# lbcb-sci/herro

Hardware: AMD Instinct MI355X
Metric: 4096-bp windows corrected/sec at batch=128 (higher is better)
Workload: dtype f16; 1 GPU; synthetic windows, 4096 bp, 32 overlaps each, batch=128, 1xMI355X per rank (BASELINE configs[2]); batch=128, window=4096, overlaps=32, batches_per_launch_group=32, streams_per_gpu=2, distinct_windows_cycled=16384, precision=5, total_windows=165760, strong_leg_windows=0

## Files before the change

herro_amd/csrc/pileup.hip:

```cpp
#include <hip/hip_runtime.h>
#include <stdint.h>

#include <cstdio>
#include <cstdlib>
#include <mutex>
#include <set>
#include <type_traits>

#include "job_dev.h"
#include "pileup_core.h"

namespace herro {

namespace {

constexpr uint32_t NONE = 0xffffffffu;
constexpr uint32_t RF_LEFT = 0x80000000u;
constexpr uint32_t ROWCAP = HERRO_TILE;
constexpr uint32_t SCAP = 128;
constexpr uint32_t QEVCAP = 2048;

template <int NT>
__device__ __forceinline__ uint32_t blk_scan(uint32_t v, uint32_t* total, uint32_t* s_wave ) {
  const int lane = threadIdx.x & 63, wave = threadIdx.x >> 6;
// ... 930 lines not shown
#pragma unroll
    for (int q = 0; q < 5; q++) cw[q] = cg == 0 ? cnt8[q][0] : (cg == 1 ? cnt8[q][1] : (cg == 2 ? cnt8[q][2] : cnt8[q][3]));
    const uint4 adj = *reinterpret_cast<const uint4*>(s_adj + seg * 16u + cg * 4u);
    const uint32_t adjw[4] = {adj.x, adj.y, adj.z, adj.w};
    uint32_t supb = 0, consw = 0;
#pragma unroll
    for (int q4 = 0; q4 < 4; q4++) {
      uint32_t c5[5];
#pragma unroll
      for (int q = 0; q < 4; q++) c5[q] = ((cw[q] >> (8 * q4)) & 0xffu) + ((adjw[q4] >> (5 * q)) & 31u);
      c5[4] = ((cw[4] >> (8 * q4)) & 0xffu) - (adjw[q4] >> 20);
      const uint32_t thresh = (uint32_t)((double)HERRO_ROWS * 0.1);
      uint32_t ns = 0;
#pragma unroll
      for (int q = 0; q < 5; q++) ns += c5[q] >= thresh ? 1u : 0u;
      if (ns >= 2 && seg * 16u + cg * 4u + q4 < nrows) supb |= 1u << q4;
      uint32_t c0 = c5[0], i0 = 0;
#pragma unroll
      for (uint32_t q = 1; q < 5; q++) if (c5[q] > c0) { c0 = c5[q]; i0 = q; }
      uint32_t c1 = 0, i1 = 5;
      bool have = false;
#pragma unroll
      for (uint32_t q = 0; q < 5; q++)
        if (q != i0 && (!have || c5[q] > c1)) { c1 = c5[q]; i1 = q; have = true; }
      const uint32_t tb0 = (tgw >> (q4 * 8)) & 0xffu;
      const uint32_t cons_v = (c0 < 2u || (c0 == c1 && (i0 == tb0 || i1 == tb0))) ? tb0 : i0;
      consw |= cons_v << (q4 * 8);
    }
    if (aux) *reinterpret_cast<uint32_t*>(J.cons_tmp + wd.row_off + r0 + seg * 16u + cg * 4u) = consw;
    if (supb) atomicOr(&s_supbits[(seg * 16u + cg * 4u) >> 5], supb << ((seg * 16u + cg * 4u) & 31u));
  }
  __syncthreads();
  PROF_MARK(J, 3, 5);
  if (aux && tid < 64) {
    const uint32_t bits = tid < ROWCAP / 32 ? s_supbits[tid] : 0u;
    const uint32_t inc = wscan_incl((uint32_t)__popc(bits));
    uint32_t k = inc - (uint32_t)__popc(bits);
    for (uint32_t m = bits; m; m &= m - 1u) {
      const uint32_t ric = (tid << 5) + (uint32_t)__ffs((int)m) - 1u;
      const uint32_t p = pa + (s_rowinfo[ric] & 0x7fffu), row = r0 + ric;
      J.sup_row[wd.row_off + r0 + k] = row;
      J.sup_pi[wd.row_off + r0 + k] = p | ((row - rop(p)) << 16);
      k++;
    }
    if (tid == 63) J.tile_nsup[tile] = inc;
  }
  PROF_MARK(J, 3, 6);
}

__global__ __launch_bounds__(64) void k_supgather(JobDev J) {
  const uint32_t w = blockIdx.x, lane = threadIdx.x;
  const WinDesc wd = J.win[w];
  const uint32_t Lf = J.win_Lf[w], tile0 = (uint32_t)wd.col_off;
  const uint32_t nch = (Lf + ROWCAP - 1) / ROWCAP;
  uint32_t dst = 0;
  for (uint32_t c0 = 0; c0 < nch; c0 += 64) {
    const uint32_t i = c0 + lane;
    const uint32_t cn = i < nch ? J.tile_nsup[tile0 + i] : 0u;
    const uint32_t inc = wscan_incl(cn);
    const uint32_t my_dst = dst + inc - cn;
    for (uint32_t j = 0; j < 64 && c0 + j < nch; j++) {
      const uint32_t cnt_j = (uint32_t)__builtin_amdgcn_readlane((int)cn, (int)j), dst_j = (uint32_t)__builtin_amdgcn_readlane((int)my_dst, (int)j);
      const uint32_t src = (c0 + j) * ROWCAP;
      if (src == dst_j) continue;
      for (uint32_t k = lane; k < cnt_j; k += 64) {
        const uint32_t a = J.sup_row[wd.row_off + src + k], b = J.sup_pi[wd.row_off + src + k];
        J.sup_row[wd.row_off + dst_j + k] = a;
        J.sup_pi[wd.row_off + dst_j + k] = b;
      }
    }
    dst += wlast(inc);
  }
  if (lane == 0) J.win_nsup[w] = dst;
}

#ifndef HERRO_RW_ICAP
#define HERRO_RW_ICAP 2048
#endif
constexpr uint32_t RW_ICAP = HERRO_RW_ICAP;
#define RI(p) ((p) + ((p) >> 5))
__host__ __device__ inline size_t rows_lds(uint32_t W) { return (size_t)(W + 2 + ((W + 2) >> 5) + 1) * 4; }

constexpr uint32_t RW_SUPCAP = 256;
template <int SP>
__device__ __forceinline__ void rf_slot(const JobDev& J, const CTab* __restrict__ s_ct, const WinDesc& wd, uint32_t Lf, uint32_t half, uint32_t c,
                                        uint32_t srow, uint32_t pj, uint32_t nr, bool have_nr, uint4* __restrict__ out);

template <int NW>
__global__ __launch_bounds__(2 * NW) void k_rows(JobDev J) {
  constexpr int NT = 2 * NW;
  extern __shared__ __attribute__((aligned(16))) uint32_t rw_smem[];
  uint32_t* s_rop = rw_smem;
  uint32_t* s_mrg = rw_smem + rows_lds(J.window_size) / 4;
  __shared__ __attribute__((aligned(16))) CTab s_ct[32];
  __shared__ uint32_t s_adj[RW_ICAP];
  __shared__ __attribute__((aligned(16))) uint8_t s_iv[RW_ICAP];
  __shared__ uint32_t s_rfbase;
  __shared__ uint32_t s_sup[3][RW_SUPCAP];
  __shared__ uint32_t s_wave[NT / 64];
  const uint32_t w = blockIdx.x, tid = threadIdx.x, nw = J.nw;
  const uint32_t half = tid >= (uint32_t)NW ? 1u : 0u, lt = tid - half * NW;
  PROF_BEGIN(J);
  const WinDesc wd = J.win[w];
  const uint32_t Lf = J.win_Lf[w], win_len = wd.win_len;
  const uint32_t tile0 = (uint32_t)wd.col_off;
  {
    constexpr int RL = 17;
    uint32_t rv[RL];
    const uint32_t* __restrict__ rop = J.row_of_pos2 + wd.pos_off;
#pragma unroll
    for (int u = 0; u < RL; u++) rv[u] = rop[min(tid + (uint32_t)u * NT, win_len)];
    if (tid < 32) s_ct[tid] = J.ctab[(uint64_t)w * 32 + tid];
#pragma unroll
    for (int u = 0; u < RL; u++) {
      const uint32_t p = tid + (uint32_t)u * NT;
      if (p <= win_len) s_rop[RI(p)] = rv[u];
    }
  }
  __syncthreads();
  PROF_MARK(J, 6, 0);
  const bool active = lt < nw;
  const uint32_t widx = min(lt, nw - 1u);
  const int32_t P = (int32_t)(widx << 5);
  const uint32_t vm = active ? mask_range(0, (int32_t)win_len - P) : 0u;
  const uint64_t pmax = J.read_n_words + 1;
  const uint32_t tlo = glb_bits(J.read_p0, s_ct[0].q_woff, pmax, (int32_t)wd.tstart + P) & vm;
  const uint32_t thi = glb_bits(J.read_p1, s_ct[0].q_woff, pmax, (int32_t)wd.tstart + P) & vm;
  uint32_t c0[5], c1[5];
  uint32_t nin[5];
  const uint32_t tsym[4] = {vm & ~tlo & ~thi, tlo & ~thi, thi & ~tlo, tlo & thi};
#pragma unroll
  for (int q = 0; q < 4; q++) { c0[q] = half ? 0u : tsym[q]; c1[q] = 0; }
  c0[4] = 0; c1[4] = 0;
  nin[0] = half ? 0u : vm; nin[1] = 0; nin[2] = 0; nin[3] = 0; nin[4] = 0;
  auto sat_add = [&](int q, uint32_t x) { sat2_add(c0[q], c1[q], x); };
  {
    constexpr int UB = 15;
    const uint32_t cb = 1u + UB * half;
    uint32_t M[UB], L[UB], H[UB];
#pragma unroll
    for (int u = 0; u < UB; u++) {
      const uint32_t o = s_ct[cb + u].ow;
      const PlaneRec g = J.cw[(o != NONE ? (uint64_t)o : 0ull) * nw + widx];
      M[u] = g.m; L[u] = g.lo; H[u] = g.hi;
    }
    PROF_MARK(J, 6, 10);
#pragma unroll
    for (int u = 0; u < UB; u++) {
      const CTab& h = s_ct[cb + u];
      const uint32_t tt = h.ow != NONE ? h.t_total : 0u;
      const uint32_t inr = mask_range(h.off - P, h.off + (int32_t)tt - P) & vm;
      const uint32_t Mi = M[u] & inr, Li = L[u] & Mi, Hi = H[u] & Mi;
      sat_add(0, Mi & ~Li & ~Hi);
      sat_add(1, Li & ~Hi);
      sat_add(2, Hi & ~Li);
      sat_add(3, Li & Hi);
      sat_add(4, inr & ~Mi);
      uint32_t x = inr;
#pragma unroll
      for (int b = 0; b < 5; b++) { const uint32_t cy = nin[b] & x; nin[b] ^= x; x = cy; }
    }
  }
  if (half) {
#pragma unroll
    for (int q = 0; q < 5; q++) { s_mrg[(q) * NW + lt] = c0[q]; s_mrg[(5 + q) * NW + lt] = c1[q]; s_mrg[(10 + q) * NW + lt] = nin[q]; }
  }
  __syncthreads();
  if (!half) {
#pragma unroll
    for (int q = 0; q < 5; q++) sat2_merge(c0[q], c1[q], s_mrg[q * NW + lt], s_mrg[(5 + q) * NW + lt]);
    uint32_t cy = 0;
#pragma unroll
    for (int b = 0; b < 5; b++) {
      const uint32_t x = nin[b], y = s_mrg[(10 + b) * NW + lt];
      nin[b] = x ^ y ^ cy;
      cy = (x & y) | (cy & (x ^ y));
    }
  }
  const bool lane0 = !half && active;
  constexpr uint32_t IP_ROWS = (RW_ICAP * 2 + NW * 4 - 1) / (NW * 4);
  static_assert(IP_ROWS + 7 <= 15, "s_mrg holds the insertion rows' positions, five cover planes and two words per lane");
  uint16_t* s_ip = reinterpret_cast<uint16_t*>(s_mrg);
// ... 73 lines not shown
            if (s_ct[c].sdir < 0) code ^= 3u;
          }
          atomicAdd(&s_adj[ir], (1u << (5u * code)) + (inr ? 1u << 20 : 0u));
          s_ip[ir] = (uint16_t)p;
        }
      }
    }
    __syncthreads();
    PROF_MARK(J, 6, 8);
    for (uint32_t i = tid; i < min(RW_ICAP, n_irows - ch0); i += NT) {
      const uint32_t adj = s_adj[i];
      uint32_t cover = 0, p = 0;
      if (adj) {
        p = s_ip[i];
        const uint32_t pw = p >> 5, pb = p & 31u;
        cover = ((s_nin[pw] >> pb) & 1u) | (((s_nin[NW + pw] >> pb) & 1u) << 1) | (((s_nin[2 * NW + pw] >> pb) & 1u) << 2) |
                (((s_nin[3 * NW + pw] >> pb) & 1u) << 3) | (((s_nin[4 * NW + pw] >> pb) & 1u) << 4);
      }
      const uint32_t c5[5] = {adj & 31u, (adj >> 5) & 31u, (adj >> 10) & 31u, (adj >> 15) & 31u, cover - (adj >> 20)};
      uint32_t ns = 0;
#pragma unroll
      for (int q = 0; q < 5; q++) ns += c5[q] >= 3u ? 1u : 0u;
      s_iv[i] = (uint8_t)(vote5(c5, 4u) | ((ns >= 2u ? 1u : 0u) << 7));
      if (ns >= 2u) { atomicOr(&s_insup[p >> 5], 1u << (p & 31u)); atomicAdd(&s_nisup[p >> 5], 1u); }
    }
    __syncthreads();
    PROF_MARK(J, 6, 9);
    if (lane0) { insup = s_insup[lt]; n_isup = s_nisup[lt]; }
    {
      const uint32_t nb = min(RW_ICAP, n_irows - ch0);
      uint32_t* __restrict__ dst = reinterpret_cast<uint32_t*>(J.cons_tmp + wd.row_off + ch0);
      for (uint32_t i = tid; i * 4u < nb; i += NT) dst[i] = reinterpret_cast<const uint32_t*>(s_iv)[i];
    }
  }
  PROF_MARK(J, 6, 3);
  const bool iv_lds = n_irows <= RW_ICAP;
  if (!iv_lds) __syncthreads();
  uint32_t total;
  uint32_t kk = blk_scan<NT>((uint32_t)__popc(supb) + n_isup, &total, s_wave);
  for (uint32_t m = supb | insup; m; m &= m - 1u) {
    const uint32_t k = (uint32_t)__ffs((int)m) - 1u, p = (uint32_t)P + k;
    const uint32_t rp = s_rop[RI(p)];
    uint32_t nr = 0;
#pragma unroll
    for (int i = 0; i < 4; i++) {
      const int32_t q = (int32_t)p - 2 + i;
      if (q >= 0 && q < (int32_t)win_len) nr |= (s_rop[RI((uint32_t)q + 1u)] - s_rop[RI((uint32_t)q)]) << (6 * i);
    }
    if ((supb >> k) & 1u) {
      J.sup_row[wd.row_off + kk] = rp;
      J.sup_pi[wd.row_off + kk] = p;
      J.sup_nr[wd.row_off + kk] = nr;
      if (kk < RW_SUPCAP) { s_sup[0][kk] = rp; s_sup[1][kk] = p; s_sup[2][kk] = nr; }
      kk++;
    }
    if ((insup >> k) & 1u) {
      const uint32_t n_ins = s_rop[RI(p + 1)] - rp - 1u;
      for (uint32_t j = 0; j < n_ins; j++) {
        const uint32_t ir = rp - p + j;
        uint32_t fl;
        if (iv_lds) fl = (uint32_t)s_iv[ir]; else fl = (uint32_t)J.cons_tmp[wd.row_off + ir];
        if (fl & 0x80u) {
          J.sup_row[wd.row_off + kk] = rp + 1u + j;
          J.sup_pi[wd.row_off + kk] = p | ((j + 1u) << 16);
          J.sup_nr[wd.row_off + kk] = nr;
          if (kk < RW_SUPCAP) { s_sup[0][kk] = rp + 1u + j; s_sup[1][kk] = p | ((j + 1u) << 16); s_sup[2][kk] = nr; }
          kk++;
        }
      }
    }
  }
  if (tid == 0) J.win_nsup[w] = total;
  PROF_MARK(J, 6, 4);
  if (J.rf) {
    if (tid == 0) {
      const uint32_t base = atomicAdd(J.rf_alloc, total);
      const bool room = (uint64_t)base + total <= J.rf_cap, ok = room && total <= RW_SUPCAP;
      s_rfbase = ok ? base : NONE;
      J.win_rfbase[w] = ok ? base : (room ? (base | RF_LEFT) : NONE);
    }
    __syncthreads();
    const uint32_t base = s_rfbase;
    if (base != NONE) {
      const uint32_t nslots = total * HERRO_ROWS;
      for (uint32_t sl = tid; sl < nslots; sl += NT) {
        const uint32_t k = sl / HERRO_ROWS, c = sl - k * HERRO_ROWS;
        uint4* __restrict__ out = reinterpret_cast<uint4*>(J.rf + ((uint64_t)base * HERRO_ROWS + sl) * 16);
        if (J.rf_half <= 2u) rf_slot<5>(J, s_ct, wd, Lf, J.rf_half, c, s_sup[0][k], s_sup[1][k], s_sup[2][k], true, out);
        else rf_slot<8>(J, s_ct, wd, Lf, J.rf_half, c, s_sup[0][k], s_sup[1][k], s_sup[2][k], true, out);
      }
    }
    PROF_MARK(J, 6, 5);
  }
}

constexpr int PQ_NT = 256;
constexpr uint32_t RFCAP = 1024;
__host__ __device__ inline size_t quals_lds(uint32_t nw) {
  return (size_t)(HERRO_ROWS - 1) * nw * 4 + (((size_t)(HERRO_ROWS - 1) * nw * 2 + 15) & ~(size_t)15) + (size_t)QEVCAP * 8;
}

template <bool FULL>
__global__ __launch_bounds__(PQ_NT) void k_quals(JobDev J, uint32_t half) {
  extern __shared__ __attribute__((aligned(16))) unsigned char pq_smem[];
  const uint32_t nw = J.nw;
  uint32_t* s_M = reinterpret_cast<uint32_t*>(pq_smem);
  uint16_t* s_rk = reinterpret_cast<uint16_t*>(s_M + (size_t)(HERRO_ROWS - 1) * nw);
  uint2* s_ev = reinterpret_cast<uint2*>(pq_smem + (size_t)(HERRO_ROWS - 1) * nw * 4 + (((size_t)(HERRO_ROWS - 1) * nw * 2 + 15) & ~(size_t)15));
  __shared__ __attribute__((aligned(16))) CTab s_ct[32];
  __shared__ uint32_t s_evl[33];
  __shared__ uint32_t s_rm[RFCAP];
  __shared__ uint32_t s_rr[RFCAP];
  const uint32_t w = blockIdx.x, tid = threadIdx.x, lane = tid & 63u, wave = tid >> 6;
  const uint32_t nsup = J.win_nsup[w], Lf = J.win_Lf[w];
  const WinDesc wd = J.win[w];
  if (tid < 32) s_ct[tid] = J.ctab[(uint64_t)w * 32 + tid];
  if (!FULL && !nsup) return;
  __syncthreads();
  if (tid < 64) {
    const uint32_t ne = (tid >= 1 && tid < 32) ? s_ct[tid].n_ev : 0u;
    const uint32_t inc = wscan_incl(ne);
    if (tid < 32) s_evl[tid] = inc - ne;
    if (tid == 31) s_evl[32] = inc;
  }
  __syncthreads();
  const uint32_t n_events = s_evl[32];
  const bool ev_in_lds = n_events <= QEVCAP;
  const uint32_t span = 2 * half + 1;
  const uint32_t kper = max(1u, RFCAP / span);
  {
    const uint32_t items = (HERRO_ROWS - 1) * nw;
    constexpr int MI = 16;
    uint32_t srow = 0;
    if (!FULL && tid < min(kper, nsup)) srow = J.sup_row[wd.row_off + tid];
    constexpr int EI = QEVCAP / PQ_NT;
    uint2 ev[EI];
    if (ev_in_lds) {
#pragma unroll
      for (int u = 0; u < EI; u++) {
        const uint32_t e = min(tid + u * PQ_NT, n_events ? n_events - 1u : 0u);
        uint32_t lo = 0, hi = 32;
        while (hi - lo > 1) {
          const uint32_t mid = (lo + hi) >> 1;
          if (s_evl[mid] <= e) lo = mid; else hi = mid;
        }
        ev[u] = n_events ? *reinterpret_cast<const uint2*>(J.iev + (uint64_t)s_ct[lo].ev_off + (e - s_evl[lo])) : make_uint2(0, 0);
      }
    }
    for (uint32_t it0 = tid; it0 < items; it0 += MI * PQ_NT) {
      uint32_t mv[MI];
#pragma unroll
      for (int u = 0; u < MI; u++) {
        const uint32_t it = min(it0 + u * PQ_NT, items - 1u);
        const uint32_t c = it / nw, wi = it - c * nw;
        const uint32_t o = s_ct[c + 1].ow;
        mv[u] = J.cw[(o != NONE ? (uint64_t)o : 0ull) * nw + wi].m;
      }
#pragma unroll
      for (int u = 0; u < MI; u++) {
        const uint32_t it = it0 + u * PQ_NT;
        if (it < items) s_M[it] = s_ct[it / nw + 1].ow != NONE ? mv[u] : 0u;
      }
    }
    if (ev_in_lds) {
#pragma unroll
      for (int u = 0; u < EI; u++) if (tid + u * PQ_NT < n_events) s_ev[tid + u * PQ_NT] = ev[u];
    }
    if (!FULL && tid < min(kper, nsup)) s_rr[tid] = srow;
  }
  __syncthreads();
  uint32_t pre_rm = NONE, pre_r = 0;
  const bool pre = !FULL && kper <= PQ_NT && min(kper, nsup) * span <= PQ_NT * 1u;
  if (pre) {
// ... 57 lines not shown
      bool found = false;
      qi = 0;
      while (i > 0) {
        const uint32_t ex = ev_x(i - 1);
        if ((ex & 0xffffu) != p) break;
        if ((ex >> 16) >= j) { qi = ev_y(i - 1) + j - 1u; found = true; break; }
        i--;
      }
      if (!found) return NONE64;
    }
    const int64_t si = (int64_t)q.sbase + (int64_t)q.sdir * (int64_t)qi;
    return min(q.qual_off + (uint64_t)max(si, (int64_t)0), qmax);
  };
  auto run = [&](auto evlds) {
    if (FULL) {
      const uint64_t total = (uint64_t)Lf * HERRO_ROWS;
      for (uint64_t idx0 = tid; idx0 < total; idx0 += 4 * PQ_NT) {
        uint32_t rm[4];
        uint64_t dst[4], src[4];
        uint32_t cc[4];
#pragma unroll
        for (int u = 0; u < 4; u++) {
          const uint64_t idx = min(idx0 + (uint64_t)u * PQ_NT, total - 1);
          cc[u] = (uint32_t)(idx / Lf);
          const uint32_t r = (uint32_t)(idx - (uint64_t)cc[u] * Lf);
          rm[u] = J.rowmap2[wd.row_off + r];
          dst[u] = wd.fin_off + (uint64_t)cc[u] * wd.lub + r;
        }
#pragma unroll
        for (int u = 0; u < 4; u++) src[u] = cell_addr(evlds, cc[u], rm[u] & 0xffffu, rm[u] >> 16);
        uint32_t qv[4];
#pragma unroll
        for (int u = 0; u < 4; u++) qv[u] = J.read_qual[src[u] == NONE64 ? 0 : src[u]];
#pragma unroll
        for (int u = 0; u < 4; u++)
          if (idx0 + (uint64_t)u * PQ_NT < total) J.fin_q[dst[u]] = (uint8_t)(src[u] == NONE64 ? 33u : qv[u]);
      }
    } else {
      for (uint32_t k0 = 0; k0 < nsup; k0 += kper) {
        const uint32_t nk = min(kper, nsup - k0), nrows = nk * span;
        if (k0 == 0 && pre) {
          if (tid < nrows) { s_rr[tid] = pre_r; s_rm[tid] = pre_rm; }
        } else {
          __syncthreads();
          for (uint32_t i = tid; i < nrows; i += PQ_NT) {
            const int64_t r = (int64_t)J.sup_row[wd.row_off + k0 + i / span] + (int64_t)(i % span) - (int64_t)half;
            const bool in = r >= 0 && r < (int64_t)Lf;
            s_rr[i] = (uint32_t)r;
            s_rm[i] = in ? J.rowmap2[wd.row_off + (uint32_t)r] : NONE;
          }
        }
        __syncthreads();
        const uint32_t total = nrows * HERRO_ROWS;
        uint8_t* __restrict__ outp = J.fin_q;
        constexpr int CB = 10;
        for (uint32_t idx0 = tid; idx0 < total; idx0 += CB * PQ_NT) {
          uint64_t dst[CB], src[CB];
          bool live[CB];
#pragma unroll
          for (int u = 0; u < CB; u++) {
            const uint32_t idx = min(idx0 + u * PQ_NT, total - 1u);
            const uint32_t slot = idx / HERRO_ROWS, c = idx - slot * HERRO_ROWS;
            dst[u] = wd.fin_off + (uint64_t)c * wd.lub + s_rr[slot];
            const uint32_t rm = s_rm[slot];
            live[u] = idx0 + u * PQ_NT < total && rm != NONE;
            src[u] = live[u] ? cell_addr(evlds, c, rm & 0xffffu, rm >> 16) : NONE64;
          }
          uint32_t qv[CB];
#pragma unroll
          for (int u = 0; u < CB; u++) qv[u] = J.read_qual[src[u] == NONE64 ? 0 : src[u]];
#pragma unroll
          for (int u = 0; u < CB; u++)
            if (live[u]) outp[dst[u]] = (uint8_t)(src[u] == NONE64 ? 33u : qv[u]);
        }
      }
    }
  };
  if (ev_in_lds) run(std::true_type{}); else run(std::false_type{});
}

constexpr int RQ_NT = 512;

template <int SP>
__device__ __forceinline__ void rf_slot(const JobDev& J, const CTab* __restrict__ s_ct, const WinDesc& wd, uint32_t Lf, uint32_t half, uint32_t c,
                                        uint32_t srow, uint32_t pj, uint32_t nr, bool have_nr, uint4* __restrict__ out) {
  const uint32_t nw = J.nw;
  const uint32_t span = 2 * half + 1, win_len = wd.win_len;
  const uint64_t tq_off = s_ct[0].qual_off + wd.tstart;
  const uint64_t qmax = J.read_qual_bytes ? J.read_qual_bytes - 1 : 0;
  const uint64_t pmax = J.read_n_words + 1;
  constexpr uint64_t NONE64 = ~0ull;
  const uint32_t* __restrict__ rop = J.row_of_pos2 + wd.pos_off;
  const int32_t pc = (int32_t)(pj & 0xffffu);
  const int64_t row0 = (int64_t)srow - (int64_t)half;
  uint32_t rv[SP];
  if (have_nr && half == 2) {
    const uint32_t rc = srow - (pj >> 16);
    rv[2] = rc;
    rv[1] = rc - ((nr >> 6) & 63u);
    rv[0] = rv[1] - (nr & 63u);
    rv[3] = rc + ((nr >> 12) & 63u);
    rv[4] = rv[3] + ((nr >> 18) & 63u);
    if constexpr (SP > 5) { rv[5] = 0; rv[6] = 0; rv[7] = 0; }
  } else {
#pragma unroll
    for (int i = 0; i < SP; i++) rv[i] = rop[(uint32_t)min(max(pc - (int32_t)half + i, 0), (int32_t)win_len)];
  }
  uint32_t rm[SP];
#pragma unroll
  for (int d = 0; d < SP; d++) {
    const int64_t r = row0 + d;
    rm[d] = NONE;
    if ((uint32_t)d < span && r >= 0 && r < (int64_t)Lf) {
      int32_t pp = 0;
      uint32_t rb = 0;
#pragma unroll
      for (int i = 0; i < SP; i++) {
        const int32_t q = pc - (int32_t)half + i;
        if ((uint32_t)i <= 2 * half && q >= 0 && q < (int32_t)win_len && (int64_t)rv[i] <= r) { pp = q; rb = rv[i]; }
      }
      rm[d] = (uint32_t)pp | (((uint32_t)r - rb) << 16);
    }
  }
  uint64_t addr[SP];
  uint32_t tok[SP];
#pragma unroll
  for (int d = 0; d < SP; d++) { addr[d] = NONE64; tok[d] = TOK_NONE; }
  const CTab& q = s_ct[c];
  if (c == 0) {
    const uint64_t tw = s_ct[0].q_woff;
#pragma unroll
    for (int d = 0; d < SP; d++) {
      if (rm[d] == NONE) continue;
      tok[d] = TOK_GAP_F;
      if ((rm[d] >> 16) == 0) {
        const uint32_t tp = wd.tstart + (rm[d] & 0xffffu);
        const uint64_t wi = min(tw + (tp >> 5), pmax);
        addr[d] = min(tq_off + (rm[d] & 0xffffu), qmax);
        tok[d] = ((J.read_p0[wi] >> (tp & 31u)) & 1u) | (((J.read_p1[wi] >> (tp & 31u)) & 1u) << 1);
      }
    }
  } else if (q.ow != NONE) {
    const uint32_t tbase = q.tokc & 0xffu, tgap = q.tokc >> 8;
    uint32_t p0 = NONE;
#pragma unroll
    for (int d = SP - 1; d >= 0; d--) if (rm[d] != NONE) p0 = rm[d] & 0xffffu;
    if (p0 != NONE) {
      const uint32_t w0 = min(p0 >> 5, nw - 1u), w1 = min(w0 + 1u, nw - 1u);
      const PlaneRec* __restrict__ cw = J.cw + (uint64_t)q.ow * nw;
      const uint32_t* __restrict__ cwd = J.cwd + (uint64_t)q.ow * nw;
      const PlaneRec c0 = cw[w0], c1 = cw[w1];
      uint2 dd;
      __builtin_memcpy(&dd, cwd + w0, 8);
      const uint2 d0 = make_uint2(c0.m, dd.x), d1 = make_uint2(c1.m, w1 != w0 ? dd.y : dd.x);
      const uint32_t l0 = c0.lo, l1 = c1.lo, h0 = c0.hi, h1 = c1.hi;
      const uint32_t m0 = d0.x, m1 = d1.x;
      const uint32_t n_ev = q.n_ev;
      const uint4* __restrict__ iev = J.iev + q.ev_off;
      uint32_t qw = d0.y & 0xfffffu, e = d0.y >> 20;
      if (d0.y == 0xffffffffu) {
        qw = 0; e = 0;
        for (uint32_t i = 0; i < w0; i++) qw += (uint32_t)__popc(cw[i].m);
        while (e < n_ev && (iev[e].x & 0xffffu) < (w0 << 5)) { qw += iev[e].x >> 16; e++; }
      }
      uint32_t pl = p0;
      bool ins_row = false;
#pragma unroll
      for (int d = 0; d < SP; d++) if (rm[d] != NONE) { pl = rm[d] & 0xffffu; ins_row = ins_row || (rm[d] >> 16) != 0; }
      const bool quiet = d0.y != 0xffffffffu && d1.y != 0xffffffffu && w1 != w0 && (d1.y >> 20) == e && (pl >> 5) == w0 && !ins_row;
      const uint32_t e_first = e;
      const uint4 none4 = make_uint4(0xffffffffu, 0, 0, 0);
      const uint32_t e_last = n_ev ? n_ev - 1u : 0u;
      uint4 ep0 = iev[min(e, e_last)], ep1 = iev[min(e + 1u, e_last)], ep2 = iev[min(e + 2u, e_last)], ep3 = iev[min(e + 3u, e_last)];
      if (quiet || e >= n_ev) ep0.x = 0xffffffffu;
      if (quiet || e + 1u >= n_ev) ep1.x = 0xffffffffu;
      if (quiet || e + 2u >= n_ev) ep2.x = 0xffffffffu;
      if (quiet || e + 3u >= n_ev) ep3.x = 0xffffffffu;
      auto ev_at = [&](uint32_t i) -> uint4 {
        if (i >= n_ev) return none4;
        const uint32_t o = i - e_first;
        if (o >= 4u) return iev[i];
        const uint4 a = (o & 1u) ? ep1 : ep0, b = (o & 1u) ? ep3 : ep2;
        return (o & 2u) ? b : a;
      };
      uint4 ecur = ep0;
      uint32_t cum = 0;
#pragma unroll
      for (int d = 0; d < SP; d++) {
        if (rm[d] == NONE) continue;
        const uint32_t p = rm[d] & 0xffffu, j = rm[d] >> 16;
        while ((ecur.x & 0xffffu) < p) {
          cum += ecur.x >> 16;
          e++;
          ecur = ev_at(e);
        }
        const bool second = (p >> 5) != w0;
        const uint32_t mw = second ? m1 : m0;
        const uint32_t below = (uint32_t)__popc(mw & ((1u << (p & 31u)) - 1u)) + (second ? (uint32_t)__popc(m0) : 0u);
        const uint32_t mbit = (mw >> (p & 31u)) & 1u;
        const bool inr = p - (uint32_t)q.off < q.t_total;
        uint32_t qi = NONE;
        tok[d] = inr ? tgap : (uint32_t)TOK_NONE;
        if (j == 0) {
          if (inr && mbit) {
            qi = qw + below + cum;
            tok[d] = tbase + ((((second ? l1 : l0) >> (p & 31u)) & 1u) | ((((second ? h1 : h0) >> (p & 31u)) & 1u) << 1));
          }
        } else if ((ecur.x & 0xffffu) == p) {
          uint4 x = ecur;
          uint32_t code = 0;
          for (uint32_t i = e;;) {
            if ((x.x >> 16) >= j) {
              qi = x.y + j - 1u;
              code = j <= 16u ? (((x.z >> (j - 1u)) & 1u) | (((x.z >> (15u + j)) & 1u) << 1)) : 4u;
            }
            if (++i >= n_ev) break;
            x = ev_at(i);
            if ((x.x & 0xffffu) != p) break;
          }
          if (qi != NONE) {
            if (code == 4u) {
              const int32_t si = q.sbase + q.sdir * (int32_t)qi;
              const uint64_t wi = min(q.q_woff + ((uint32_t)si >> 5), pmax);
              code = ((J.read_p0[wi] >> ((uint32_t)si & 31u)) & 1u) | (((J.read_p1[wi] >> ((uint32_t)si & 31u)) & 1u) << 1);
              if (q.sdir < 0) code ^= 3u;
            }
            tok[d] = tbase + code;
          }
        }
        if (qi != NONE) {
          const int64_t si = (int64_t)q.sbase + (int64_t)q.sdir * (int64_t)qi;
          addr[d] = min(q.qual_off + (uint64_t)max(si, (int64_t)0), qmax);
        }
      }
    }
  }
  uint32_t qv[SP];
#pragma unroll
  for (int d = 0; d < SP; d++) qv[d] = J.read_qual[addr[d] == NONE64 ? 0 : addr[d]];
  uint32_t lo = 0, hi = 0, tl = 0, th = 0;
#pragma unroll
  for (int d = 0; d < 4; d++) {
    lo |= (addr[d] == NONE64 ? 33u : qv[d]) << (8 * d);
    tl |= tok[d] << (8 * d);
    if (d + 4 < SP) {
      hi |= (addr[(d + 4) % SP] == NONE64 ? 33u : qv[(d + 4) % SP]) << (8 * d);
      th |= tok[(d + 4) % SP] << (8 * d);
    } else {
      hi |= 33u << (8 * d);
      th |= (uint32_t)TOK_NONE << (8 * d);
    }
  }
  *out = make_uint4(tl, th, lo, hi);
}

template <int SP>
__global__ __launch_bounds__(RQ_NT) void k_rfq(JobDev J, uint32_t half, const uint64_t* __restrict__ sup_off, uint8_t* __restrict__ rf, uint64_t cap, uint32_t have_nr) {
  __shared__ __attribute__((aligned(16))) CTab s_ct[32];
  const uint32_t w = gridDim.x - 1u - blockIdx.x, tid = threadIdx.x;
  PROF_BEGIN(J);
  const uint32_t nsup = J.win_nsup[w], Lf = J.win_Lf[w];
  const bool left_only = (have_nr & 2u) != 0u;
  have_nr &= 1u;
  uint64_t slot0;
  if (left_only) {
    const uint32_t rb = J.win_rfbase[w];
    if (!nsup || rb == NONE || !(rb & RF_LEFT)) return;
    slot0 = rb & ~RF_LEFT;
  } else {
    if (!nsup || sup_off[w] + nsup > cap) return;
    slot0 = sup_off[w];
  }
  const WinDesc wd = J.win[w];
  if (tid < 32) s_ct[tid] = J.ctab[(uint64_t)w * 32 + tid];
  __syncthreads();
  PROF_MARK(J, 5, 0);
  const uint32_t nslots = nsup * HERRO_ROWS;
  const uint64_t out0 = slot0 * HERRO_ROWS;
  for (uint32_t sl = tid; sl < nslots; sl += RQ_NT) {
    const uint32_t k = sl / HERRO_ROWS, c = sl - k * HERRO_ROWS;
    const uint32_t pj = J.sup_pi[wd.row_off + k], srow = J.sup_row[wd.row_off + k];
    const uint32_t nr = have_nr ? J.sup_nr[wd.row_off + k] : 0u;
    rf_slot<SP>(J, s_ct, wd, Lf, half, c, srow, pj, nr, have_nr != 0u, reinterpret_cast<uint4*>(rf + (out0 + sl) * 16));
    PROF_MARK(J, 5, 1);
  }
}

constexpr int PC_NT = 256;
__global__ __launch_bounds__(PC_NT) void k_consensus(JobDev J, const uint64_t* sup_off, const float* base_logits) {
  __shared__ uint32_t s_wave[PC_NT / 64];
  const uint32_t w = blockIdx.x;
  const WinDesc wd = J.win[w];
  const uint32_t Lf = J.win_Lf[w], n_kept = J.win_nkept[w];
  const uint32_t n_alns = n_kept < 30u ? n_kept : 30u;
  uint8_t* seq = J.cons_seq + wd.row_off;
  if (n_alns < 2) {
    if (threadIdx.x == 0) J.cons_len[w] = 0;
    return;
  }
  const float* lg = base_logits + sup_off[w] * 5;
  uint8_t* tmp = J.cons_tmp + wd.row_off;
  const uint32_t nsup = J.win_nsup[w];
  for (uint32_t k = threadIdx.x; k < nsup; k += PC_NT) {
    const float* l5 = lg + (uint64_t)k * 5;
    uint32_t arg = 0;
    float mx = l5[0];
#pragma unroll
    for (uint32_t c = 1; c < 5; c++) {
      const float v = l5[c];
      const bool ge = (v != v) ? true : ((mx != mx) ? false : v >= mx);
      if (ge) { arg = c; mx = v; }
    }
    tmp[J.sup_row[wd.row_off + k]] = (uint8_t)arg;
  }
  __syncthreads();
  const uint32_t ch = (Lf + PC_NT - 1) / PC_NT;
  const uint32_t a = min(threadIdx.x * ch, Lf), b = min(a + ch, Lf);
  uint32_t nout = 0;
  for (uint32_t r = a; r < b; r++) nout += tmp[r] != 4u ? 1u : 0u;
  uint32_t total;
  uint32_t o = blk_scan<PC_NT>(nout, &total, s_wave);
  uint32_t acc = 0, nacc = 0;
  for (uint32_t r = a; r < b; r++) {
    const uint32_t base = tmp[r];
    if (base == 4u) continue;
    const uint32_t ch = ((0x54474341u >> (8u * base)) & 0xffu);
    if ((o & 3u) != 0 && nacc == 0) { seq[o++] = (uint8_t)ch; continue; }
    acc |= ch << (8 * nacc);
    if (++nacc == 4) { *reinterpret_cast<uint32_t*>(seq + o) = acc; o += 4; acc = 0; nacc = 0; }
  }
  for (uint32_t k = 0; k < nacc; k++) seq[o + k] = (uint8_t)(acc >> (8 * k));
  if (threadIdx.x == 0) J.cons_len[w] = total;
}

constexpr uint32_t CP_ICAP = 4096;
constexpr uint32_t CP_OCAP = 6144;
template <int NT, int SPW>
__global__ __launch_bounds__(NT) void k_consensus_p(JobDev J, const uint64_t* sup_off, const float* base_logits) {
  extern __shared__ __attribute__((aligned(16))) uint32_t cp_smem[];
  uint32_t* s_rop = cp_smem;
  __shared__ uint32_t s_v[3][HERRO_MAX_WINDOW / 32];
  __shared__ uint32_t s_im[HERRO_MAX_WINDOW / 32];
  __shared__ __attribute__((aligned(16))) uint8_t s_iv[CP_ICAP];
  __shared__ __attribute__((aligned(16))) uint8_t s_out[CP_OCAP];
  __shared__ uint32_t s_wave[NT / 64];
  const uint32_t w = blockIdx.x, tid = threadIdx.x, nw = J.nw;
  PROF_BEGIN(J);
  const WinDesc wd = J.win[w];
  const uint32_t Lf = J.win_Lf[w], n_kept = J.win_nkept[w], win_len = wd.win_len;
  const uint32_t n_alns = n_kept < 30u ? n_kept : 30u;
  uint8_t* __restrict__ seq = J.cons_seq + wd.row_off;
  if (n_alns < 2) {
    if (tid == 0) J.cons_len[w] = 0;
    return;
  }
  const uint32_t n_irows = Lf - win_len;
  const bool iv_lds = n_irows <= CP_ICAP;
  uint8_t* __restrict__ giv = J.cons_tmp + wd.row_off;
  {
    constexpr int RL = SPW == 4 ? 9 : 17;
    uint32_t rv[RL];
    const uint32_t* __restrict__ rop = J.row_of_pos2 + wd.pos_off;
#pragma unroll
    for (int u = 0; u < RL; u++) rv[u] = rop[min(tid + (uint32_t)u * NT, win_len)];
    uint32_t vv[4] = {0, 0, 0, 0};
    if (tid < nw) {
      const uint32_t* __restrict__ vp = J.vpl + (uint64_t)w * 4 * nw + tid;
      vv[0] = vp[0]; vv[1] = vp[nw]; vv[2] = vp[2 * nw]; vv[3] = vp[3 * nw];
// ... 222 lines not shown
```

Measured before the change: 3.543 million windows/s.

## Share per-row feature plans across columns via LDS in row-feature gather

Row-feature generation now runs in two phases. Each supporting row's position/row mapping (the plan) is computed once per chunk of 64 rows and stored in shared memory, and every column thread reuses it instead of recomputing it. The target column and the other columns get separate specialised paths. The per-column event walk becomes a branch-free accumulation over prefetched events, and quality loads use 32-bit offsets. This removes redundant row-mapping work and divergent loops, at the cost of extra syncthreads per chunk and LDS space reused from the merge buffer.

```diff
diff --git a/herro_amd/csrc/pileup.hip b/herro_amd/csrc/pileup.hip
--- a/herro_amd/csrc/pileup.hip
+++ b/herro_amd/csrc/pileup.hip
@@ -1036,9 +1036,11 @@
 __host__ __device__ inline size_t rows_lds(uint32_t W) { return (size_t)(W + 2 + ((W + 2) >> 5) + 1) * 4; }
 
 constexpr uint32_t RW_SUPCAP = 256;
-template <int SP>
-__device__ __forceinline__ void rf_slot(const JobDev& J, const CTab* __restrict__ s_ct, const WinDesc& wd, uint32_t Lf, uint32_t half, uint32_t c,
-                                        uint32_t srow, uint32_t pj, uint32_t nr, bool have_nr, uint4* __restrict__ out);
+constexpr uint32_t RF_CHUNK = 64;
+constexpr uint32_t rf_pw(int SP) { return (uint32_t)((SP + 2 + 3) & ~3); }
+template <int SP, int NT, class RowSrc>
+__device__ __forceinline__ void rf_window(const JobDev& J, const CTab* __restrict__ s_ct, uint32_t* __restrict__ s_plan, const WinDesc& wd, uint32_t Lf, uint32_t half,
+                                          bool have_nr, uint32_t nsup, uint8_t* __restrict__ rf, uint64_t slot0, RowSrc rows);
 
 template <int NW>
 __global__ __launch_bounds__(2 * NW) void k_rows(JobDev J) {
@@ -1052,6 +1054,8 @@
   __shared__ uint32_t s_rfbase;
   __shared__ uint32_t s_sup[3][RW_SUPCAP];
   __shared__ uint32_t s_wave[NT / 64];
+  static_assert(15 * NW >= (int)(RF_CHUNK * rf_pw(8)) + 3, "s_mrg holds a chunk of row plans");
+  uint32_t* s_plan = rw_smem + ((rows_lds(J.window_size) / 4 + 3) & ~(size_t)3);
   const uint32_t w = blockIdx.x, tid = threadIdx.x, nw = J.nw;
   const uint32_t half = tid >= (uint32_t)NW ? 1u : 0u, lt = tid - half * NW;
   PROF_BEGIN(J);
@@ -1291,13 +1295,9 @@
     __syncthreads();
     const uint32_t base = s_rfbase;
     if (base != NONE) {
-      const uint32_t nslots = total * HERRO_ROWS;
-      for (uint32_t sl = tid; sl < nslots; sl += NT) {
-        const uint32_t k = sl / HERRO_ROWS, c = sl - k * HERRO_ROWS;
-        uint4* __restrict__ out = reinterpret_cast<uint4*>(J.rf + ((uint64_t)base * HERRO_ROWS + sl) * 16);
-        if (J.rf_half <= 2u) rf_slot<5>(J, s_ct, wd, Lf, J.rf_half, c, s_sup[0][k], s_sup[1][k], s_sup[2][k], true, out);
-        else rf_slot<8>(J, s_ct, wd, Lf, J.rf_half, c, s_sup[0][k], s_sup[1][k], s_sup[2][k], true, out);
-      }
+      auto rows = [&](uint32_t k, uint32_t& srow, uint32_t& pj, uint32_t& nr) { srow = s_sup[0][k]; pj = s_sup[1][k]; nr = s_sup[2][k]; };
+      if (J.rf_half <= 2u) rf_window<5, NT>(J, s_ct, s_plan, wd, Lf, J.rf_half, true, total, J.rf, base, rows);
+      else rf_window<8, NT>(J, s_ct, s_plan, wd, Lf, J.rf_half, true, total, J.rf, base, rows);
     }
     PROF_MARK(J, 6, 5);
   }
@@ -1521,14 +1521,10 @@
 constexpr int RQ_NT = 512;
 
 template <int SP>
-__device__ __forceinline__ void rf_slot(const JobDev& J, const CTab* __restrict__ s_ct, const WinDesc& wd, uint32_t Lf, uint32_t half, uint32_t c,
-                                        uint32_t srow, uint32_t pj, uint32_t nr, bool have_nr, uint4* __restrict__ out) {
+__device__ __forceinline__ void rf_plan(const JobDev& J, const WinDesc& wd, uint32_t Lf, uint32_t half, uint32_t srow, uint32_t pj, uint32_t nr, bool have_nr,
+                                        uint32_t* __restrict__ plan) {
   const uint32_t nw = J.nw;
   const uint32_t span = 2 * half + 1, win_len = wd.win_len;
-  const uint64_t tq_off = s_ct[0].qual_off + wd.tstart;
-  const uint64_t qmax = J.read_qual_bytes ? J.read_qual_bytes - 1 : 0;
-  const uint64_t pmax = J.read_n_words + 1;
-  constexpr uint64_t NONE64 = ~0ull;
   const uint32_t* __restrict__ rop = J.row_of_pos2 + wd.pos_off;
   const int32_t pc = (int32_t)(pj & 0xffffu);
   const int64_t row0 = (int64_t)srow - (int64_t)half;
@@ -1561,129 +1557,40 @@
       rm[d] = (uint32_t)pp | (((uint32_t)r - rb) << 16);
     }
   }
-  uint64_t addr[SP];
-  uint32_t tok[SP];
-#pragma unroll
-  for (int d = 0; d < SP; d++) { addr[d] = NONE64; tok[d] = TOK_NONE; }
-  const CTab& q = s_ct[c];
-  if (c == 0) {
-    const uint64_t tw = s_ct[0].q_woff;
-#pragma unroll
-    for (int d = 0; d < SP; d++) {
-      if (rm[d] == NONE) continue;
-      tok[d] = TOK_GAP_F;
-      if ((rm[d] >> 16) == 0) {
-        const uint32_t tp = wd.tstart + (rm[d] & 0xffffu);
-        const uint64_t wi = min(tw + (tp >> 5), pmax);
-        addr[d] = min(tq_off + (rm[d] & 0xffffu), qmax);
-        tok[d] = ((J.read_p0[wi] >> (tp & 31u)) & 1u) | (((J.read_p1[wi] >> (tp & 31u)) & 1u) << 1);
-      }
-    }
-  } else if (q.ow != NONE) {
-    const uint32_t tbase = q.tokc & 0xffu, tgap = q.tokc >> 8;
-    uint32_t p0 = NONE;
-#pragma unroll
-    for (int d = SP - 1; d >= 0; d--) if (rm[d] != NONE) p0 = rm[d] & 0xffffu;
-    if (p0 != NONE) {
-      const uint32_t w0 = min(p0 >> 5, nw - 1u), w1 = min(w0 + 1u, nw - 1u);
-      const PlaneRec* __restrict__ cw = J.cw + (uint64_t)q.ow * nw;
-      const uint32_t* __restrict__ cwd = J.cwd + (uint64_t)q.ow * nw;
-      const PlaneRec c0 = cw[w0], c1 = cw[w1];
-      uint2 dd;
-      __builtin_memcpy(&dd, cwd + w0, 8);
-      const uint2 d0 = make_uint2(c0.m, dd.x), d1 = make_uint2(c1.m, w1 != w0 ? dd.y : dd.x);
-      const uint32_t l0 = c0.lo, l1 = c1.lo, h0 = c0.hi, h1 = c1.hi;
-      const uint32_t m0 = d0.x, m1 = d1.x;
-      const uint32_t n_ev = q.n_ev;
-      const uint4* __restrict__ iev = J.iev + q.ev_off;
-      uint32_t qw = d0.y & 0xfffffu, e = d0.y >> 20;
-      if (d0.y == 0xffffffffu) {
-        qw = 0; e = 0;
-        for (uint32_t i = 0; i < w0; i++) qw += (uint32_t)__popc(cw[i].m);
-        while (e < n_ev && (iev[e].x & 0xffffu) < (w0 << 5)) { qw += iev[e].x >> 16; e++; }
-      }
-      uint32_t pl = p0;
-      bool ins_row = false;
-#pragma unroll
-      for (int d = 0; d < SP; d++) if (rm[d] != NONE) { pl = rm[d] & 0xffffu; ins_row = ins_row || (rm[d] >> 16) != 0; }
-      const bool quiet = d0.y != 0xffffffffu && d1.y != 0xffffffffu && w1 != w0 && (d1.y >> 20) == e && (pl >> 5) == w0 && !ins_row;
-      const uint32_t e_first = e;
-      const uint4 none4 = make_uint4(0xffffffffu, 0, 0, 0);
-      const uint32_t e_last = n_ev ? n_ev - 1u : 0u;
-      uint4 ep0 = iev[min(e, e_last)], ep1 = iev[min(e + 1u, e_last)], ep2 = iev[min(e + 2u, e_last)], ep3 = iev[min(e + 3u, e_last)];
-      if (quiet || e >= n_ev) ep0.x = 0xffffffffu;
-      if (quiet || e + 1u >= n_ev) ep1.x = 0xffffffffu;
-      if (quiet || e + 2u >= n_ev) ep2.x = 0xffffffffu;
-      if (quiet || e + 3u >= n_ev) ep3.x = 0xffffffffu;
-      auto ev_at = [&](uint32_t i) -> uint4 {
-        if (i >= n_ev) return none4;
-        const uint32_t o = i - e_first;
-        if (o >= 4u) return iev[i];
-        const uint4 a = (o & 1u) ? ep1 : ep0, b = (o & 1u) ? ep3 : ep2;
-        return (o & 2u) ? b : a;
-      };
-      uint4 ecur = ep0;
-      uint32_t cum = 0;
-#pragma unroll
-      for (int d = 0; d < SP; d++) {
-        if (rm[d] == NONE) continue;
-        const uint32_t p = rm[d] & 0xffffu, j = rm[d] >> 16;
-        while ((ecur.x & 0xffffu) < p) {
-          cum += ecur.x >> 16;
-          e++;
-          ecur = ev_at(e);
-        }
-        const bool second = (p >> 5) != w0;
-        const uint32_t mw = second ? m1 : m0;
-        const uint32_t below = (uint32_t)__popc(mw & ((1u << (p & 31u)) - 1u)) + (second ? (uint32_t)__popc(m0) : 0u);
-        const uint32_t mbit = (mw >> (p & 31u)) & 1u;
-        const bool inr = p - (uint32_t)q.off < q.t_total;
-        uint32_t qi = NONE;
-        tok[d] = inr ? tgap : (uint32_t)TOK_NONE;
-        if (j == 0) {
-          if (inr && mbit) {
-            qi = qw + below + cum;
-            tok[d] = tbase + ((((second ? l1 : l0) >> (p & 31u)) & 1u) | ((((second ? h1 : h0) >> (p & 31u)) & 1u) << 1));
-          }
-        } else if ((ecur.x & 0xffffu) == p) {
-          uint4 x = ecur;
-          uint32_t code = 0;
-          for (uint32_t i = e;;) {
-            if ((x.x >> 16) >= j) {
-              qi = x.y + j - 1u;
-              code = j <= 16u ? (((x.z >> (j - 1u)) & 1u) | (((x.z >> (15u + j)) & 1u) << 1)) : 4u;
-            }
-            if (++i >= n_ev) break;
-            x = ev_at(i);
-            if ((x.x & 0xffffu) != p) break;
-          }
-          if (qi != NONE) {
-            if (code == 4u) {
-              const int32_t si = q.sbase + q.sdir * (int32_t)qi;
-              const uint64_t wi = min(q.q_woff + ((uint32_t)si >> 5), pmax);
-              code = ((J.read_p0[wi] >> ((uint32_t)si & 31u)) & 1u) | (((J.read_p1[wi] >> ((uint32_t)si & 31u)) & 1u) << 1);
-              if (q.sdir < 0) code ^= 3u;
-            }
-            tok[d] = tbase + code;
-          }
-        }
-        if (qi != NONE) {
-          const int64_t si = (int64_t)q.sbase + (int64_t)q.sdir * (int64_t)qi;
-          addr[d] = min(q.qual_off + (uint64_t)max(si, (int64_t)0), qmax);
-        }
-      }
-    }
-  }
-  uint32_t qv[SP];
-#pragma unroll
-  for (int d = 0; d < SP; d++) qv[d] = J.read_qual[addr[d] == NONE64 ? 0 : addr[d]];
+  uint32_t p0 = 0, pl = 0, rows = 0, ins = 0;
+#pragma unroll
+  for (int d = SP - 1; d >= 0; d--) if (rm[d] != NONE) p0 = rm[d] & 0xffffu;
+#pragma unroll
+  for (int d = 0; d < SP; d++)
+    if (rm[d] != NONE) { pl = rm[d] & 0xffffu; rows |= 1u << d; ins |= (rm[d] >> 16) != 0 ? 1u : 0u; }
+  const uint32_t w0 = min(p0 >> 5, nw - 1u), w1 = min(w0 + 1u, nw - 1u);
+  uint32_t second = 0;
+#pragma unroll
+  for (int d = 0; d < SP; d++) if (rm[d] != NONE && ((rm[d] & 0xffffu) >> 5) != w0) second |= 1u << d;
+#pragma unroll
+  for (int d = 0; d < SP; d++) plan[d] = rm[d] != NONE ? rm[d] : 0u;
+  plan[SP] = p0 | (ins << 15) | (pl << 16);
+  plan[SP + 1] = w0 | (w1 << 8) | (rows << 16) | (second << 24);
+}
+
+template <int SP>
+__device__ __forceinline__ void rf_load_plan(const uint32_t* __restrict__ plan, uint32_t (&pw)[rf_pw(SP)]) {
+#pragma unroll
+  for (int i = 0; i < (int)rf_pw(SP); i += 4) {
+    const uint4 v = *reinterpret_cast<const uint4*>(plan + i);
+    pw[i] = v.x; pw[i + 1] = v.y; pw[i + 2] = v.z; pw[i + 3] = v.w;
+  }
+}
+
+template <int SP>
+__device__ __forceinline__ void rf_store(const uint32_t (&tok)[SP], const uint32_t (&qv)[SP], uint32_t has, uint4* __restrict__ out) {
   uint32_t lo = 0, hi = 0, tl = 0, th = 0;
 #pragma unroll
   for (int d = 0; d < 4; d++) {
-    lo |= (addr[d] == NONE64 ? 33u : qv[d]) << (8 * d);
+    lo |= ((has >> d) & 1u ? qv[d] : 33u) << (8 * d);
     tl |= tok[d] << (8 * d);
     if (d + 4 < SP) {
-      hi |= (addr[(d + 4) % SP] == NONE64 ? 33u : qv[(d + 4) % SP]) << (8 * d);
+      hi |= ((has >> (d + 4)) & 1u ? qv[(d + 4) % SP] : 33u) << (8 * d);
       th |= tok[(d + 4) % SP] << (8 * d);
     } else {
       hi |= 33u << (8 * d);
@@ -1694,8 +1601,156 @@
 }
 
 template <int SP>
+__device__ __forceinline__ void rf_target(const JobDev& J, const CTab& t0, const WinDesc& wd, const uint32_t* __restrict__ plan, uint4* __restrict__ out) {
+  const uint64_t tq_off = t0.qual_off + wd.tstart, tw = t0.q_woff;
+  const uint64_t qmax = J.read_qual_bytes ? J.read_qual_bytes - 1 : 0;
+  const uint64_t pmax = J.read_n_words + 1;
+  uint32_t pw[rf_pw(SP)];
+  rf_load_plan<SP>(plan, pw);
+  const uint32_t rows = (pw[SP + 1] >> 16) & 0xffu;
+  uint64_t addr[SP];
+  uint32_t tok[SP], has = 0;
+#pragma unroll
+  for (int d = 0; d < SP; d++) {
+    addr[d] = 0;
+    tok[d] = TOK_NONE;
+    if (!((rows >> d) & 1u)) continue;
+    tok[d] = TOK_GAP_F;
+    if ((pw[d] >> 16) == 0) {
+      const uint32_t tp = wd.tstart + (pw[d] & 0xffffu);
+      const uint64_t wi = min(tw + (tp >> 5), pmax);
+      addr[d] = min(tq_off + (pw[d] & 0xffffu), qmax);
+      has |= 1u << d;
+      tok[d] = ((J.read_p0[wi] >> (tp & 31u)) & 1u) | (((J.read_p1[wi] >> (tp & 31u)) & 1u) << 1);
+    }
+  }
+  uint32_t qv[SP];
+#pragma unroll
+  for (int d = 0; d < SP; d++) qv[d] = J.read_qual[addr[d]];
+  rf_store<SP>(tok, qv, has, out);
+}
+
+template <int SP>
+__device__ __forceinline__ void rf_col(const JobDev& J, const CTab& q, const uint32_t* __restrict__ plan, uint4* __restrict__ out) {
+  const uint32_t nw = J.nw;
+  const uint64_t qmax = J.read_qual_bytes ? J.read_qual_bytes - 1 : 0;
+  const uint64_t pmax = J.read_n_words + 1;
+  uint32_t pw[rf_pw(SP)];
+  rf_load_plan<SP>(plan, pw);
+  const uint32_t rows = (pw[SP + 1] >> 16) & 0xffu;
+  uint32_t tok[SP], qo[SP], has = 0;
+#pragma unroll
+  for (int d = 0; d < SP; d++) { tok[d] = TOK_NONE; qo[d] = 0; }
+  if (q.ow != NONE) {
+    if (rows != 0u) {
+      const uint32_t tbase = q.tokc & 0xffu, tgap = q.tokc >> 8;
+      const uint32_t w0 = pw[SP + 1] & 0xffu, w1 = (pw[SP + 1] >> 8) & 0xffu, pl = pw[SP] >> 16, second = pw[SP + 1] >> 24;
+      const PlaneRec* __restrict__ cw = J.cw + (uint64_t)q.ow * nw;
+      const uint32_t* __restrict__ cwd = J.cwd + (uint64_t)q.ow * nw;
+      const PlaneRec c0 = cw[w0], c1 = cw[w1];
+      const uint32_t dy = cwd[w0];
+      const uint32_t l0 = c0.lo, l1 = c1.lo, h0 = c0.hi, h1 = c1.hi;
+      const uint32_t m0 = c0.m, m1 = c1.m;
+      const uint32_t n_ev = q.n_ev;
+      const uint4* __restrict__ iev = J.iev + q.ev_off;
+      uint32_t qw = dy & 0xfffffu, e = dy >> 20;
+      if (dy == 0xffffffffu) {
+        qw = 0; e = 0;
+        for (uint32_t i = 0; i < w0; i++) qw += (uint32_t)__popc(cw[i].m);
+        while (e < n_ev && (iev[e].x & 0xffffu) < (w0 << 5)) { qw += iev[e].x >> 16; e++; }
+      }
+      uint32_t p[SP], jm1[SP];
+      uint32_t cum[SP];
+      uint32_t ey[SP], ez[SP];
+#pragma unroll
+      for (int d = 0; d < SP; d++) { p[d] = pw[d] & 0xffffu; jm1[d] = (pw[d] >> 16) - 1u; cum[d] = 0; ey[d] = NONE; ez[d] = 0; }
+      auto apply = [&](const uint4& x, bool there) {
+        const uint32_t xp = there ? (x.x & 0xffffu) : 0xffffu, xl = x.x >> 16;
+#pragma unroll
+        for (int d = 0; d < SP; d++) {
+          cum[d] += xp < p[d] ? xl : 0u;
+          const bool wrote = xp == p[d] && jm1[d] < xl;
+          ey[d] = wrote ? x.y : ey[d];
+          ez[d] = wrote ? x.z : ez[d];
+        }
+      };
+      const uint32_t e_last = n_ev ? n_ev - 1u : 0u;
+      const uint4 ep0 = iev[min(e, e_last)], ep1 = iev[min(e + 1u, e_last)], ep2 = iev[min(e + 2u, e_last)], ep3 = iev[min(e + 3u, e_last)];
+      apply(ep0, e < n_ev);
+      apply(ep1, e + 1u < n_ev);
+      apply(ep2, e + 2u < n_ev);
+      apply(ep3, e + 3u < n_ev);
+      if (e + 4u < n_ev && (ep3.x & 0xffffu) <= pl)
+        for (uint32_t i = e + 4u; i < n_ev; i++) {
+          const uint4 x = iev[i];
+          if ((x.x & 0xffffu) > pl) break;
+          apply(x, true);
+        }
+#pragma unroll
+      for (int d = 0; d < SP; d++) {
+        const bool mine = ((rows >> d) & 1u) != 0u, sec = ((second >> d) & 1u) != 0u, base_row = jm1[d] == NONE;
+        const uint32_t sh = p[d] & 31u;
+        const uint32_t mw = sec ? m1 : m0;
+        const uint32_t below = (uint32_t)__popc(mw & ((1u << sh) - 1u)) + (sec ? (uint32_t)__popc(m0) : 0u);
+        const uint32_t mbit = (mw >> sh) & 1u;
+        const bool inr = p[d] - (uint32_t)q.off < q.t_total;
+        const uint32_t bcode = (((sec ? l1 : l0) >> sh) & 1u) | ((((sec ? h1 : h0) >> sh) & 1u) << 1);
+        const bool based = base_row && inr && mbit != 0u;
+        const bool insd = !base_row && ey[d] != NONE;
+        uint32_t icode = ((ez[d] >> (jm1[d] & 31u)) & 1u) | (((ez[d] >> ((jm1[d] + 16u) & 31u)) & 1u) << 1);
+        const uint32_t qi = based ? qw + below + cum[d] : ey[d] + jm1[d];
+        if (insd && jm1[d] >= 16u) {
+          const int32_t si = q.sbase + q.sdir * (int32_t)qi;
+          const uint64_t wi = min(q.q_woff + ((uint32_t)si >> 5), pmax);
+          icode = ((J.read_p0[wi] >> ((uint32_t)si & 31u)) & 1u) | (((J.read_p1[wi] >> ((uint32_t)si & 31u)) & 1u) << 1);
+          if (q.sdir < 0) icode ^= 3u;
+        }
+        const uint32_t t = based ? tbase + bcode : insd ? tbase + icode : inr ? tgap : (uint32_t)TOK_NONE;
+        tok[d] = mine ? t : (uint32_t)TOK_NONE;
+        if (mine && (based || insd)) {
+          has |= 1u << d;
+          qo[d] = (uint32_t)max(q.sbase + q.sdir * (int32_t)qi, 0);
+        }
+      }
+    }
+  }
+  const uint64_t qb = min(q.qual_off, qmax);
+  const uint32_t qlim = (uint32_t)min(qmax - qb, (uint64_t)0x7fffffffu);
+  const uint8_t* __restrict__ rq = J.read_qual + qb;
+  uint32_t qv[SP];
+#pragma unroll
+  for (int d = 0; d < SP; d++) qv[d] = rq[min(qo[d], qlim)];
+  rf_store<SP>(tok, qv, has, out);
+}
+
+template <int SP, int NT, class RowSrc>
+__device__ __forceinline__ void rf_window(const JobDev& J, const CTab* __restrict__ s_ct, uint32_t* __restrict__ s_plan, const WinDesc& wd, uint32_t Lf, uint32_t half,
+                                          bool have_nr, uint32_t nsup, uint8_t* __restrict__ rf, uint64_t slot0, RowSrc rows) {
+  constexpr uint32_t PW = rf_pw(SP), NC = HERRO_ROWS - 1;
+  const uint32_t tid = threadIdx.x;
+  for (uint32_t k0 = 0; k0 < nsup; k0 += RF_CHUNK) {
+    const uint32_t n = min(nsup - k0, RF_CHUNK);
+    if (k0) __syncthreads();
+    if (tid < n) {
+      uint32_t srow, pj, nr;
+      rows(k0 + tid, srow, pj, nr);
+      rf_plan<SP>(J, wd, Lf, half, srow, pj, nr, have_nr, s_plan + tid * PW);
+    }
+    __syncthreads();
+    uint4* __restrict__ out = reinterpret_cast<uint4*>(rf + (slot0 + k0) * HERRO_ROWS * 16);
+    const uint32_t tl = (uint32_t)NT - 1u - tid;
+    if (tl < n) rf_target<SP>(J, s_ct[0], wd, s_plan + tl * PW, out + tl * HERRO_ROWS);
+    for (uint32_t sl = tid; sl < n * NC; sl += NT) {
+      const uint32_t k = sl / NC, c = 1u + sl - k * NC;
+      rf_col<SP>(J, s_ct[c], s_plan + k * PW, out + k * HERRO_ROWS + c);
+    }
+  }
+}
+
+template <int SP>
 __global__ __launch_bounds__(RQ_NT) void k_rfq(JobDev J, uint32_t half, const uint64_t* __restrict__ sup_off, uint8_t* __restrict__ rf, uint64_t cap, uint32_t have_nr) {
   __shared__ __attribute__((aligned(16))) CTab s_ct[32];
+  __shared__ __attribute__((aligned(16))) uint32_t s_plan[RF_CHUNK * rf_pw(SP)];
   const uint32_t w = gridDim.x - 1u - blockIdx.x, tid = threadIdx.x;
   PROF_BEGIN(J);
   const uint32_t nsup = J.win_nsup[w], Lf = J.win_Lf[w];
@@ -1714,15 +1769,14 @@
   if (tid < 32) s_ct[tid] = J.ctab[(uint64_t)w * 32 + tid];
   __syncthreads();
   PROF_MARK(J, 5, 0);
-  const uint32_t nslots = nsup * HERRO_ROWS;
-  const uint64_t out0 = slot0 * HERRO_ROWS;
-  for (uint32_t sl = tid; sl < nslots; sl += RQ_NT) {
-    const uint32_t k = sl / HERRO_ROWS, c = sl - k * HERRO_ROWS;
-    const uint32_t pj = J.sup_pi[wd.row_off + k], srow = J.sup_row[wd.row_off + k];
-    const uint32_t nr = have_nr ? J.sup_nr[wd.row_off + k] : 0u;
-    rf_slot<SP>(J, s_ct, wd, Lf, half, c, srow, pj, nr, have_nr != 0u, reinterpret_cast<uint4*>(rf + (out0 + sl) * 16));
-    PROF_MARK(J, 5, 1);
-  }
+  auto rows = [&](uint32_t k, uint32_t& srow, uint32_t& pj, uint32_t& nr) {
+    pj = J.sup_pi[wd.row_off + k];
+    srow = J.sup_row[wd.row_off + k];
+    nr = 0u;
+    if (have_nr) nr = J.sup_nr[wd.row_off + k];
+  };
+  rf_window<SP, RQ_NT>(J, s_ct, s_plan, wd, Lf, half, have_nr != 0u, nsup, rf, slot0, rows);
+  PROF_MARK(J, 5, 1);
 }
 
 constexpr int PC_NT = 256;
```

Measured after the change: 3.531 million windows/s (median of 3 runs). No clear change (-0.3%).
